# tugitbartlomiej/ViTParticleFilterTracker

Hardware: AMD Instinct MI355X
Metric: frames/sec @ 4096 particles, ViT-B/16 224px; 1/2/4/8 MI355X scaling (higher is better)
Workload: dtype bf16; 1 GPU; 4096 particles, vit_base_patch16_224 bf16, 224x224 frames, full tracking step per frame; particles=4096, particles_per_gpu=4096, arch=vit_base_patch16_224, hip_graph=True, parallelism=particle-shard x1

## Files before the change

### vitparticlefiltertracker_amd/csrc/gemm_bf16.hip

```cpp
#include <algorithm>
#include "gemm_common.h"

using namespace vpf;
using namespace vpf::gemm;

namespace {

constexpr int BK = 64;
constexpr int OPERAND_BYTES = BM * BK * 2;
static_assert(OPERAND_BYTES == TILE_BYTES, "bf16 K-tile geometry");
constexpr int AUX_PARTS = 15;
constexpr int MAX_PARTS = 16;
constexpr int AUX_BYTES = 2048 + AUX_PARTS * 2048;

template <int EPI, bool WIDE = false, bool OUT8 = false, bool PART = false>
__global__ __launch_bounds__(NTHREADS) void k_gemm_bf16(const bf16_t* __restrict__ A, int lda,
                                                        const bf16_t* __restrict__ W,
                                                        const float* __restrict__ bias,
                                                        const bf16_t* residual,
                                                        const float* __restrict__ pos, int g2,
                                                        const float2* __restrict__ stats,
                                                        const float* __restrict__ colsum,
                                                        bf16_t* C, int ldc, int M, int N, int K, int group,
                                                        int stats_parts, float ln_eps, float* stats_out,
                                                        int stats_rows, Out8 o8) {
    constexpr int SMEM = 5 * OPERAND_BYTES;
    static_assert(AUX_BYTES <= OPERAND_BYTES, "aux region must fit the free A slot of the deep ring");
    __shared__ __attribute__((aligned(16))) char smem[SMEM];
    const int tid = threadIdx.x, lane = tid & 63;
    const int wid = __builtin_amdgcn_readfirstlane(tid >> 6);

    int m0, n0;
    tile_of(M, N, group, m0, n0);
    constexpr bool DIRECT = (EPI == VPF_EPI_LN_GELU || EPI == VPF_EPI_BIAS_GELU) && !OUT8 && !PART;

    const int kbase = PART ? (int)blockIdx.y * (K / (int)gridDim.y) : 0;
    const char* Ablk = reinterpret_cast<const char*>(A) + (size_t)m0 * lda * 2 + (size_t)kbase * 2;
    const char* Bblk = reinterpret_cast<const char*>(W) + (size_t)n0 * K * 2 + (size_t)kbase * 2;
    uint32_t offA[4], offB[4];
#pragma unroll
    for (int i = 0; i < 4; ++i) {
        const int g = i * 8 + wid;
        const int row = 8 * g + (lane >> 3);
        const int pch = lane & 7;
        const int lch = pch ^ ((row >> 1) & 7);
        const int ra = min(row, M - 1 - m0);
        const int rb = min(DIRECT ? wperm(row) : row, N - 1 - n0);
        offA[i] = (uint32_t)ra * (uint32_t)(lda * 2) + (uint32_t)(lch * 16);
        offB[i] = (uint32_t)rb * (uint32_t)(K * 2) + (uint32_t)(lch * 16);
    }
    auto stage_a = [&](int kt) {
        char* la = smem + (kt % 3) * OPERAND_BYTES;
        const uint32_t koff = (uint32_t)kt * (BK * 2);
#pragma unroll
        for (int i = 0; i < 4; ++i)
            __builtin_amdgcn_global_load_lds((gptr_t)(Ablk + offA[i] + koff), (lptr_t)(la + (i * 8 + wid) * 1024), 16, 0, 0);
    };
    auto stage_b = [&](int kt) {
        char* lb = smem + (3 + (kt & 1)) * OPERAND_BYTES;
        const uint32_t koff = (uint32_t)kt * (BK * 2);
#pragma unroll
        for (int i = 0; i < 4; ++i)
            __builtin_amdgcn_global_load_lds((gptr_t)(Bblk + offB[i] + koff), (lptr_t)(lb + (i * 8 + wid) * 1024), 16, 0, 0);
    };

    const int wm = wid >> 2, wn = wid & 3;
    f32x4 acc[4][8];
#pragma unroll
    for (int j = 0; j < 4; ++j)
#pragma unroll
        for (int i = 0; i < 8; ++i) acc[j][i] = f32x4{0.f, 0.f, 0.f, 0.f};

    const int fr = lane & 15, fq = lane >> 4;

    constexpr bool LN = (EPI == VPF_EPI_LN || EPI == VPF_EPI_LN_GELU) && !PART;
    const int nk = (PART ? K / (int)gridDim.y : K) / BK;
    char* aux = smem + (nk % 3) * OPERAND_BYTES;
    constexpr bool wide = LN && WIDE;
    char* planes_lds = wide ? smem + ((nk + 1) % 3) * OPERAND_BYTES : aux + 2048;
    auto load_planes = [&](char* dst) {
        const int lane = opaque_lane();
        const float* sd = reinterpret_cast<const float*>(stats);
        const int planes = stats_parts > 0 ? stats_parts : 1;
        if ((M & 1) == 0 && ((uintptr_t)sd & 15) == 0) {
            for (int pc = wid; pc < 2 * planes; pc += 8) {
                const int p = pc >> 1, hf = pc & 1;
                __builtin_amdgcn_global_load_lds(
                    (gptr_t)(sd + (int64_t)p * 2 * M + min(2 * m0 + hf * 256 + lane * 4, 2 * M - 4)),
                    (lptr_t)(dst + p * 2048 + hf * 1024), 16, 0, 0);
            }
        } else {
            for (int p = 0; p < planes; ++p)
                __builtin_amdgcn_global_load_lds(
                    (gptr_t)(sd + (int64_t)p * 2 * M + min(2 * m0 + wid * 64 + lane, 2 * M - 1)),
                    (lptr_t)(dst + p * 2048 + wid * 256), 4, 0, 0);
        }
    };
    auto load_aux = [&]() {
        if constexpr (PART) return;
        const int lane = opaque_lane();
        if (wid == 0)
            __builtin_amdgcn_global_load_lds((gptr_t)(bias + min(n0 + lane * 4, N - 4)), (lptr_t)aux, 16, 0, 0);
        if constexpr (LN) {
            if (wid == 1)
                __builtin_amdgcn_global_load_lds((gptr_t)(colsum + min(n0 + lane * 4, N - 4)), (lptr_t)(aux + 1024), 16,
                                                 0, 0);
            if (!wide) load_planes(aux + 2048);
        }
    };
    stage_a(0);
    stage_b(0);
    if (nk > 1) stage_a(1);
    if (nk == 1) load_aux();
    for (int kt = 0; kt < nk; ++kt) {
        if (kt + 1 < nk) asm volatile("s_waitcnt vmcnt(4)" ::: "memory");
        else asm volatile("s_waitcnt vmcnt(0)" ::: "memory");
        __builtin_amdgcn_s_barrier();
        asm volatile("" ::: "memory");
        if (nk >= 2 && kt == nk - 2) load_aux();
        if (wide && kt == nk - 1) load_planes(planes_lds);
        const char* la = smem + (kt % 3) * OPERAND_BYTES;
        const char* lb = smem + (3 + (kt & 1)) * OPERAND_BYTES;
        bf16x8 a[2][8], b[2][4];
#pragma unroll
        for (int ks = 0; ks < 2; ++ks) {
#pragma unroll
            for (int j = 0; j < 4; ++j) {
                const int row = wn * 64 + j * 16 + fr;
                const int ch = (ks * 4 + fq) ^ ((row >> 1) & 7);
                b[ks][j] = *reinterpret_cast<const bf16x8*>(lb + row * 128 + ch * 16);
            }
#pragma unroll
            for (int i = 0; i < 8; ++i) {
                const int row = wm * 128 + i * 16 + fr;
                const int ch = (ks * 4 + fq) ^ ((row >> 1) & 7);
                a[ks][i] = *reinterpret_cast<const bf16x8*>(la + row * 128 + ch * 16);
            }
        }
        stage_b(min(kt + 1, nk - 1));
        stage_a(min(kt + 2, nk - 1));
#pragma unroll
        for (int ks = 0; ks < 2; ++ks)
#pragma unroll
            for (int j = 0; j < 4; ++j)
#pragma unroll
                for (int i = 0; i < 8; ++i)
                    acc[j][i] = __builtin_amdgcn_mfma_f32_16x16x32_bf16(b[ks][j], a[ks][i], acc[j][i], 0, 0, 0);
        __builtin_amdgcn_sched_group_barrier(0x100, 24, 0);
        __builtin_amdgcn_sched_group_barrier(0x020, 4, 0);
#pragma unroll
        for (int q = 0; q < 4; ++q) {
            __builtin_amdgcn_sched_group_barrier(0x008, 16, 0);
            __builtin_amdgcn_sched_group_barrier(0x020, 1, 0);
        }
    }

    if constexpr (PART) {
        __builtin_amdgcn_s_waitcnt(0x0F70);
        float* P = reinterpret_cast<float*>(C) + (size_t)blockIdx.y * M * N;
#pragma unroll
        for (int i = 0; i < 8; ++i) {
            const int m = m0 + wm * 128 + i * 16 + fr;
#pragma unroll
            for (int j = 0; j < 4; ++j) {
                const int n = n0 + wn * 64 + j * 16 + fq * 4;
                if (m < M && n < N) *reinterpret_cast<f32x4*>(P + (size_t)m * N + n) = acc[j][i];
            }
        }
        return;
    }
    if constexpr (LN) {
        if constexpr (wide) {
            asm volatile("s_waitcnt vmcnt(0)" ::: "memory");
            __builtin_amdgcn_s_barrier();
            asm volatile("" ::: "memory");
        }
        if (stats_parts > 0 && tid < BM) {
            float sm = 0.f, sq = 0.f;
            for (int p = 0; p < stats_parts; ++p) {
                const float2 st = *reinterpret_cast<const float2*>(planes_lds + p * 2048 + tid * 8);
                sm += st.x;
                sq += st.y;
            }
            const float inv_k = 1.0f / (float)K;
            const float mean = sm * inv_k;
            const float var = fmaxf(fmaf(sq, inv_k, -mean * mean), 0.f);
            *reinterpret_cast<float2*>(aux + 2048 + tid * 8) = make_float2(mean, __builtin_amdgcn_rsqf(var + ln_eps));
        }
    }
    __builtin_amdgcn_s_waitcnt(0x0F70);
    uint4 res[16];
    constexpr bool PIPE = EPI != VPF_EPI_PATCH && !OUT8;
    if constexpr (DIRECT) {
        if constexpr (LN) {
            asm volatile("s_waitcnt lgkmcnt(0)" ::: "memory");
            __builtin_amdgcn_s_barrier();
            asm volatile("" ::: "memory");
        }
        store_wave_tile_direct<EPI>(aux, acc, wm, wn, m0, n0, lane, C, ldc, M, N);
        return;
    }
    if constexpr (EPI == VPF_EPI_BIAS_RESIDUAL) load_residual<PIPE>(res, residual, wm, wn, m0, n0, lane, ldc, M, N);
    asm volatile("s_waitcnt lgkmcnt(0)" ::: "memory");
    __builtin_amdgcn_s_barrier();
    asm volatile("" ::: "memory");
    const int region = (wid >> 1) + ((wid >> 1) >= (nk % 3) ? 1 : 0);
    char* img = smem + region * OPERAND_BYTES + (wid & 1) * 16384;
    if constexpr (PIPE) {
        store_wave_tile_pipe<EPI>(img, aux, acc, wm, wn, m0, n0, lane, res, C, ldc, M, N,
                                  EPI == VPF_EPI_BIAS_RESIDUAL ? stats_out : nullptr, stats_rows);
    } else {
        float* prod_stats = (EPI == VPF_EPI_BIAS_RESIDUAL || EPI == VPF_EPI_PATCH) ? stats_out : nullptr;
        store_wave_tile<EPI, OUT8>(img, aux, acc, wm, wn, m0, n0, lane, res, pos, g2, C, ldc, M, N, prod_stats,
                                   stats_rows, o8);
    }
}

template <int EPI, bool OUT8 = false>
__global__ __launch_bounds__(NTHREADS) void k_gemm_pp(const bf16_t* __restrict__ A, int lda,
                                                      const bf16_t* __restrict__ W,
                                                      const float* __restrict__ bias,
                                                      const bf16_t* residual,
                                                      const float* __restrict__ pos, int g2,
                                                      const float2* __restrict__ stats,
                                                      const float* __restrict__ colsum,
                                                      bf16_t* C, int ldc, int M, int N, int K, int group,
                                                      int stats_parts, float ln_eps, float* stats_out,
                                                      int stats_rows, Out8 o8) {
    constexpr int HALF = 16384;
    constexpr int RING = 8 * HALF;
    static_assert(RING + AUX_BYTES <= 160 * 1024, "LDS budget");
    __shared__ __attribute__((aligned(16))) char smem[RING + AUX_BYTES];
    const int tid = threadIdx.x, lane = tid & 63;
    const int wid = __builtin_amdgcn_readfirstlane(tid >> 6);
    const int wm = wid >> 2, wn = wid & 3;

    int m0, n0;
    tile_of(M, N, group, m0, n0);
    constexpr bool DIRECT = (EPI == VPF_EPI_LN_GELU || EPI == VPF_EPI_BIAS_GELU) && !OUT8;

    const char* Ablk = reinterpret_cast<const char*>(A) + (size_t)m0 * lda * 2;
    const char* Bblk = reinterpret_cast<const char*>(W) + (size_t)n0 * K * 2;
    uint32_t off[4][2];
#pragma unroll
    for (int p = 0; p < 2; ++p) {
        const int rho = (wid + 8 * p) * 8 + (lane >> 3);
        const int lch = (lane & 7) ^ ((rho >> 1) & 7);
        const int ra0 = (rho >> 6) * 128 + (rho & 63);
        const int rb0 = (rho >> 5) * 64 + (DIRECT ? wperm(rho & 31) : (rho & 31));
        const int ra[2] = {ra0, ra0 + 64}, rb[2] = {rb0, rb0 + 32};
#pragma unroll
        for (int h = 0; h < 2; ++h) {
            off[h == 0 ? 0 : 3][p] = (uint32_t)min(ra[h], M - 1 - m0) * (uint32_t)(lda * 2) + (uint32_t)(lch * 16);
            off[h == 0 ? 1 : 2][p] = (uint32_t)min(rb[h], N - 1 - n0) * (uint32_t)(K * 2) + (uint32_t)(lch * 16);
        }
    }
    const int nk = K / BK;
    auto stage = [&](int type, int kt) {
        kt = min(kt, nk - 1);
        char* slot = smem + ((kt & 1) * 4 + type) * HALF;
        const char* src = (type == 0 || type == 3) ? Ablk : Bblk;
        const uint32_t koff = (uint32_t)kt * (BK * 2);
#pragma unroll
        for (int p = 0; p < 2; ++p)
            __builtin_amdgcn_global_load_lds((gptr_t)(src + off[type][p] + koff), (lptr_t)(slot + (wid + 8 * p) * 1024),
                                             16, 0, 0);
    };

    constexpr bool LN = (EPI == VPF_EPI_LN || EPI == VPF_EPI_LN_GELU);
    char* aux = smem + RING;
    if (wid == 0)
        __builtin_amdgcn_global_load_lds((gptr_t)(bias + min(n0 + lane * 4, N - 4)), (lptr_t)aux, 16, 0, 0);
    if constexpr (LN) {
        if (wid == 1)
            __builtin_amdgcn_global_load_lds((gptr_t)(colsum + min(n0 + lane * 4, N - 4)), (lptr_t)(aux + 1024), 16, 0, 0);
        const float* sd = reinterpret_cast<const float*>(stats);
        const int planes = stats_parts > 0 ? stats_parts : 1;
        if ((M & 1) == 0 && ((uintptr_t)sd & 15) == 0) {
            for (int pc = wid; pc < 2 * planes; pc += 8) {
                const int p = pc >> 1, hf = pc & 1;
                __builtin_amdgcn_global_load_lds((gptr_t)(sd + (int64_t)p * 2 * M + min(2 * m0 + hf * 256 + lane * 4, 2 * M - 4)),
                                                 (lptr_t)(aux + 2048 + p * 2048 + hf * 1024), 16, 0, 0);
            }
        } else {
            for (int p = 0; p < planes; ++p)
                __builtin_amdgcn_global_load_lds((gptr_t)(sd + (int64_t)p * 2 * M + min(2 * m0 + wid * 64 + lane, 2 * M - 1)),
                                                 (lptr_t)(aux + 2048 + p * 2048 + wid * 256), 4, 0, 0);
        }
    }
    stage(0, 0); stage(1, 0); stage(2, 0); stage(3, 0); stage(0, 1); stage(1, 1);
    asm volatile("s_waitcnt vmcnt(8)" ::: "memory");
    __builtin_amdgcn_s_barrier();
    if (wm == 1) __builtin_amdgcn_s_barrier();
    asm volatile("" ::: "memory");

    f32x4 acc[4][8];
#pragma unroll
    for (int j = 0; j < 4; ++j)
#pragma unroll
        for (int i = 0; i < 8; ++i) acc[j][i] = f32x4{0.f, 0.f, 0.f, 0.f};

    const int fr = lane & 15, fq = lane >> 4;
    const int sw = (fr >> 1) & 7;
    const int abase = (wm * 64 + fr) * 128, bbase = (wn * 32 + fr) * 128;
    auto mfma_quadrant = [&](const i32x4 (&fa)[2][4], const i32x4 (&fb)[2][2], int mh, int nh) {
        asm volatile("s_waitcnt lgkmcnt(0)" ::: "memory");
        __builtin_amdgcn_sched_barrier(0);
#pragma unroll
        for (int ks = 0; ks < 2; ++ks)
#pragma unroll
            for (int j = 0; j < 2; ++j)
#pragma unroll
                for (int i = 0; i < 4; ++i)
                    acc[nh * 2 + j][mh * 4 + i] = __builtin_amdgcn_mfma_f32_16x16x32_bf16(
                        __builtin_bit_cast(bf16x8, fb[ks][j]), __builtin_bit_cast(bf16x8, fa[ks][i]),
                        acc[nh * 2 + j][mh * 4 + i], 0, 0, 0);
        __builtin_amdgcn_sched_barrier(0);
    };
    auto read_a = [&](i32x4 (&fa)[2][4], const char* slot) {
#pragma unroll
        for (int ks = 0; ks < 2; ++ks)
#pragma unroll
            for (int i = 0; i < 4; ++i) fa[ks][i] = lds16(slot + abase + i * 2048 + (((ks * 4 + fq) ^ sw) << 4));
    };
    auto read_b = [&](i32x4 (&fb)[2][2], const char* slot) {
#pragma unroll
        for (int ks = 0; ks < 2; ++ks)
#pragma unroll
            for (int j = 0; j < 2; ++j) fb[ks][j] = lds16(slot + bbase + j * 2048 + (((ks * 4 + fq) ^ sw) << 4));
    };
    auto bar = [&]() {
        __builtin_amdgcn_sched_barrier(0);
        __builtin_amdgcn_s_barrier();
        __builtin_amdgcn_sched_barrier(0);
    };

    for (int kt = 0; kt < nk; ++kt) {
        const char* buf = smem + (kt & 1) * 4 * HALF;
        i32x4 fa0[2][4], fa1[2][4], fb0[2][2], fb1[2][2];
        read_a(fa0, buf);
        read_b(fb0, buf + HALF);
        stage(2, kt + 1);
        asm volatile("s_waitcnt vmcnt(8)" ::: "memory");
        bar();
        mfma_quadrant(fa0, fb0, 0, 0);
        bar();
        read_b(fb1, buf + 2 * HALF);
        stage(3, kt + 1);
        asm volatile("s_waitcnt vmcnt(8)" ::: "memory");
        bar();
        mfma_quadrant(fa0, fb1, 0, 1);
        bar();
        read_a(fa1, buf + 3 * HALF);
        stage(0, kt + 2);
        bar();
        mfma_quadrant(fa1, fb1, 1, 1);
        bar();
        stage(1, kt + 2);
        asm volatile("s_waitcnt vmcnt(8)" ::: "memory");
        bar();
        mfma_quadrant(fa1, fb0, 1, 0);
        bar();
    }
    if (wm == 0) __builtin_amdgcn_s_barrier();
    asm volatile("s_waitcnt vmcnt(0)" ::: "memory");

    if constexpr (LN) {
        if (stats_parts > 0 && tid < BM) {
            float sm = 0.f, sq = 0.f;
            for (int p = 0; p < stats_parts; ++p) {
                const float2 st = *reinterpret_cast<const float2*>(aux + 2048 + p * 2048 + tid * 8);
                sm += st.x;
                sq += st.y;
            }
            const float inv_k = 1.0f / (float)K;
            const float mean = sm * inv_k;
            const float var = fmaxf(fmaf(sq, inv_k, -mean * mean), 0.f);
            *reinterpret_cast<float2*>(aux + 2048 + tid * 8) = make_float2(mean, __builtin_amdgcn_rsqf(var + ln_eps));
        }
    }
    __builtin_amdgcn_s_waitcnt(0x0F70);
    uint4 res[16];
    constexpr bool PIPE = EPI != VPF_EPI_PATCH && !OUT8;
    if constexpr (DIRECT) {
        if constexpr (LN) {
            asm volatile("s_waitcnt lgkmcnt(0)" ::: "memory");
            __builtin_amdgcn_s_barrier();
            asm volatile("" ::: "memory");
        }
        store_wave_tile_direct<EPI>(aux, acc, wm, wn, m0, n0, lane, C, ldc, M, N);
        return;
    }
    if constexpr (EPI == VPF_EPI_BIAS_RESIDUAL) load_residual<PIPE>(res, residual, wm, wn, m0, n0, lane, ldc, M, N);
    asm volatile("s_waitcnt lgkmcnt(0)" ::: "memory");
    __builtin_amdgcn_s_barrier();
    asm volatile("" ::: "memory");
    char* img = smem + wid * 16384;
    if constexpr (PIPE) {
        store_wave_tile_pipe<EPI>(img, aux, acc, wm, wn, m0, n0, lane, res, C, ldc, M, N,
                                  EPI == VPF_EPI_BIAS_RESIDUAL ? stats_out : nullptr, stats_rows);
    } else {
        float* prod_stats = (EPI == VPF_EPI_BIAS_RESIDUAL || EPI == VPF_EPI_PATCH) ? stats_out : nullptr;
        store_wave_tile<EPI, OUT8>(img, aux, acc, wm, wn, m0, n0, lane, res, pos, g2, C, ldc, M, N, prod_stats,
                                   stats_rows, o8);
    }
}

}

#define VPF_IS_LN(E) ((E) == VPF_EPI_LN || (E) == VPF_EPI_LN_GELU)
#define VPF_IS_PROD(E) ((E) == VPF_EPI_BIAS_RESIDUAL || (E) == VPF_EPI_PATCH)
#define VPF_GEMM_ARGS                                                                                        \
    A, (int)lda, W, bias, residual, pos, patch_rows, reinterpret_cast<const float2*>(row_stats), colsum, C,     \
        (int)ldc, m, n, k, group, stats_parts, ln_eps, stats_out, stats_rows, o8
#define VPF_GEMM_LAUNCH(E)                                                                                   \
    do {                                                                                                     \
        if (kern == 5 && !(VPF_IS_LN(E) && stats_parts > AUX_PARTS) && o8.q == nullptr)                      \
            hipLaunchKernelGGL((k_gemm_pp<E, false>), grid, block, 0, s, VPF_GEMM_ARGS);                     \
        else if (kern == 5 && VPF_IS_PROD(E) && o8.q != nullptr)                                             \
            hipLaunchKernelGGL((k_gemm_pp<E, VPF_IS_PROD(E)>), grid, block, 0, s, VPF_GEMM_ARGS);            \
        else if (VPF_IS_LN(E) && stats_parts > AUX_PARTS)                                                    \
            hipLaunchKernelGGL((k_gemm_bf16<E, VPF_IS_LN(E)>), grid, block, 0, s, VPF_GEMM_ARGS);             \
        else if (VPF_IS_PROD(E) && o8.q != nullptr)                                                          \
            hipLaunchKernelGGL((k_gemm_bf16<E, false, VPF_IS_PROD(E)>), grid, block, 0, s, VPF_GEMM_ARGS);    \
        else                                                                                                 \
            hipLaunchKernelGGL((k_gemm_bf16<E>), grid, block, 0, s, VPF_GEMM_ARGS);                           \
    } while (0)

constexpr int kDefaultGroup = 4;
static int g_kernel = 0;
static int g_group = -1;
static int gemm_kernel_for(int epilogue) {
    if (g_kernel) return g_kernel;
    return (epilogue == VPF_EPI_LN || epilogue == VPF_EPI_LN_GELU) ? 5 : 1;
}
static int tile_group_for(int64_t N, int epilogue) {
    if (g_group >= 0) return g_group;
    if (N <= 1024) return 2;
    return epilogue == VPF_EPI_LN_GELU ? 8 : kDefaultGroup;
}
int vpf_gemm_tile_group() { return g_group >= 0 ? g_group : kDefaultGroup; }
int vpf_gemm_tile_group_mx8(int epilogue) {
    if (g_group >= 0) return g_group;
    return epilogue == VPF_EPI_LN ? 8 : kDefaultGroup;
}
VPF_API int vpf_gemm_tune(int kernel, int group) {
    if (kernel != 0 && kernel != 1 && kernel != 5) return VPF_ERR_ARG;
    if (group < -1 || group > 64) return VPF_ERR_ARG;
    g_kernel = kernel;
    g_group = kernel == 0 ? -1 : group;
    return 0;
}

int vpf_check_out8(const uint8_t* C8, int64_t ld8, const uint32_t* Cs, int64_t lds_c, int64_t rows, int64_t N) {
    if (!C8) return Cs ? VPF_ERR_ARG : 0;
    if (!Cs || N % 128 != 0 || ld8 < N || ld8 % 8 != 0 || ((uintptr_t)C8 & 7) || lds_c < rows || lds_c % 64 != 0 ||
        ((uintptr_t)Cs & 3) || ld8 > INT32_MAX || lds_c > INT32_MAX / 4)
        return VPF_ERR_ARG;
    return 0;
}

VPF_API int vpf_gemm_bf16(const uint16_t* A, int64_t lda, const uint16_t* W, const float* bias,
                          const uint16_t* residual, const float* pos, int patch_rows, const float* row_stats,
                          const float* colsum, uint16_t* C, int64_t ldc, int64_t M, int64_t N, int64_t K,
                          int epilogue, int stats_parts, float ln_eps, float* stats_out, uint8_t* C8, int64_t ld8,
                          uint32_t* Cs, int64_t lds_c, void* stream) {
    if (M <= 0 || N <= 0 || K <= 0 || K % BK != 0 || N % 8 != 0 || lda < K || lda % 8 != 0 || ldc < N ||
        ldc % 8 != 0)
        return VPF_ERR_ARG;
    if (M > INT32_MAX / 2 || N > 65536 || K > 65536 || lda > INT32_MAX / 2 || ldc > INT32_MAX / 2) return VPF_ERR_ARG;
    if ((uint64_t)BM * (uint64_t)lda * 2 > UINT32_MAX) return VPF_ERR_ARG;
    if (!A || !W || !bias || !C) return VPF_ERR_ARG;
    if (epilogue == VPF_EPI_BIAS_RESIDUAL && !residual) return VPF_ERR_ARG;
    if (epilogue == VPF_EPI_PATCH && (!pos || patch_rows <= 0 || M % patch_rows != 0)) return VPF_ERR_ARG;
    if ((epilogue == VPF_EPI_LN || epilogue == VPF_EPI_LN_GELU) && (!row_stats || !colsum)) return VPF_ERR_ARG;
    if (((uintptr_t)bias & 15) || ((uintptr_t)colsum & 15) || ((uintptr_t)row_stats & 7)) return VPF_ERR_ARG;
    if (stats_parts < 0 || stats_parts > MAX_PARTS || !(ln_eps >= 0.f))
        return VPF_ERR_ARG;
    if (stats_out && (((uintptr_t)stats_out & 7) || (epilogue != VPF_EPI_BIAS_RESIDUAL && epilogue != VPF_EPI_PATCH)))
        return VPF_ERR_ARG;
    const int64_t srows = epilogue == VPF_EPI_PATCH ? (M / patch_rows) * (patch_rows + 1) : M;
    if (srows > INT32_MAX) return VPF_ERR_ARG;
    const int stats_rows = (int)srows;
    if (C8 && epilogue != VPF_EPI_BIAS_RESIDUAL && epilogue != VPF_EPI_PATCH) return VPF_ERR_ARG;
    if (vpf_check_out8(C8, ld8, Cs, lds_c, srows, N)) return VPF_ERR_ARG;
    const Out8 o8{C8, reinterpret_cast<uint8_t*>(Cs), (int)ld8, (int)lds_c};
    const int64_t tiles = ((M + BM - 1) / BM) * ((N + BN - 1) / BN);
    if (tiles > INT32_MAX) return VPF_ERR_ARG;
    hipStream_t s = (hipStream_t)stream;
    const dim3 grid((unsigned)tiles), block(NTHREADS);
    const int kern = gemm_kernel_for(epilogue);
    const int group = tile_group_for(N, epilogue);
    const int m = (int)M, n = (int)N, k = (int)K;
    switch (epilogue) {
        case VPF_EPI_BIAS: VPF_GEMM_LAUNCH(VPF_EPI_BIAS); break;
        case VPF_EPI_BIAS_GELU: VPF_GEMM_LAUNCH(VPF_EPI_BIAS_GELU); break;
        case VPF_EPI_BIAS_RESIDUAL: VPF_GEMM_LAUNCH(VPF_EPI_BIAS_RESIDUAL); break;
        case VPF_EPI_PATCH: VPF_GEMM_LAUNCH(VPF_EPI_PATCH); break;
        case VPF_EPI_LN: VPF_GEMM_LAUNCH(VPF_EPI_LN); break;
        case VPF_EPI_LN_GELU: VPF_GEMM_LAUNCH(VPF_EPI_LN_GELU); break;
        default: return VPF_ERR_ARG;
    }
    VPF_RETURN_LAUNCH();
}

template <int EPI>
__global__ __launch_bounds__(256) void k_splitk_reduce(const float* __restrict__ P, int S, int M, int N,
                                                       const float* __restrict__ bias,
                                                       const float2* __restrict__ stats,
                                                       const float* __restrict__ colsum, const bf16_t* residual,
                                                       bf16_t* C, int64_t ldc, float* stats_out) {
    constexpr bool LN = (EPI == VPF_EPI_LN || EPI == VPF_EPI_LN_GELU);
    constexpr bool GELU = (EPI == VPF_EPI_BIAS_GELU || EPI == VPF_EPI_LN_GELU);
    const int per_row = N >> 3;
    const int64_t t = (int64_t)blockIdx.x * blockDim.x + threadIdx.x;
    const bool live = t < (int64_t)M * per_row;
    const int m = live ? (int)(t / per_row) : 0;
    const int n = live ? (int)(t - (int64_t)m * per_row) * 8 : 0;
    float v[8];
    if (live) {
        const float* p = P + (size_t)m * N + n;
        const float4 a0 = *reinterpret_cast<const float4*>(p), a1 = *reinterpret_cast<const float4*>(p + 4);
        v[0] = a0.x; v[1] = a0.y; v[2] = a0.z; v[3] = a0.w; v[4] = a1.x; v[5] = a1.y; v[6] = a1.z; v[7] = a1.w;
        for (int s = 1; s < S; ++s) {
            const float* q = p + (size_t)s * M * N;
            const float4 b0 = *reinterpret_cast<const float4*>(q), b1 = *reinterpret_cast<const float4*>(q + 4);
            v[0] += b0.x; v[1] += b0.y; v[2] += b0.z; v[3] += b0.w; v[4] += b1.x; v[5] += b1.y; v[6] += b1.z; v[7] += b1.w;
        }
        float rstd = 1.f, nrm = 0.f;
        if constexpr (LN) {
            const float2 st = stats[m];
            rstd = st.y;
            nrm = -st.y * st.x;
        }
#pragma unroll
        for (int e = 0; e < 8; ++e) {
            float y = LN ? fmaf(rstd, v[e], fmaf(nrm, colsum[n + e], bias[n + e])) : v[e] + bias[n + e];
            if constexpr (GELU) {
                const f32x2 g = gelu_sig2(f32x2{y, y});
                y = g.x;
            }
            v[e] = y;
        }
    }
    uint32_t o[4];
#pragma unroll
    for (int e = 0; e < 4; ++e) o[e] = pack_bf2(v[2 * e], v[2 * e + 1]);
    if constexpr (EPI == VPF_EPI_BIAS_RESIDUAL) {
        if (live) {
            const uint4 rv = *reinterpret_cast<const uint4*>(residual + (size_t)m * ldc + n);
            const uint32_t rr[4] = {rv.x, rv.y, rv.z, rv.w};
#pragma unroll
            for (int e = 0; e < 4; ++e)
                o[e] = pack_bf2(bf2f((bf16_t)(o[e] & 0xffff)) + bf2f((bf16_t)(rr[e] & 0xffff)),
                                bf2f((bf16_t)(o[e] >> 16)) + bf2f((bf16_t)(rr[e] >> 16)));
        }
        if (stats_out != nullptr) {
            float s1 = 0.f, s2 = 0.f;
            if (live) {
#pragma unroll
                for (int e = 0; e < 4; ++e) {
                    const float lo = bf2f((bf16_t)(o[e] & 0xffff)), hi = bf2f((bf16_t)(o[e] >> 16));
                    s1 += lo + hi;
                    s2 = fmaf(lo, lo, s2);
                    s2 = fmaf(hi, hi, s2);
                }
            }
#pragma unroll
            for (int x = 1; x < 8; x <<= 1) {
                s1 += __shfl_xor(s1, x, 64);
                s2 += __shfl_xor(s2, x, 64);
            }
            if (live && (n & 63) == 0)
                *reinterpret_cast<float2*>(stats_out + ((int64_t)(n >> 6) * M + m) * 2) = make_float2(s1, s2);
        }
    }
    if (live) *reinterpret_cast<uint4*>(C + (size_t)m * ldc + n) = make_uint4(o[0], o[1], o[2], o[3]);
}

VPF_API int vpf_gemm_bf16_splitk(const uint16_t* A, int64_t lda, const uint16_t* W, const float* bias,
                                 const uint16_t* residual, const float* row_stats, const float* colsum, uint16_t* C,
                                 int64_t ldc, int64_t M, int64_t N, int64_t K, int epilogue, int splits,
                                 float* stats_out, float* partial_ws, int64_t ws_elems, void* stream) {
    if (M <= 0 || N <= 0 || K <= 0 || splits < 1 || K % ((int64_t)splits * BK) != 0 || N % 8 != 0 || lda < K ||
        lda % 8 != 0 || ldc < N || ldc % 8 != 0)
        return VPF_ERR_ARG;
    if (M > INT32_MAX / 2 || N > 65536 || K > 65536 || lda > INT32_MAX / 2 || ldc > INT32_MAX / 2 || splits > 64)
        return VPF_ERR_ARG;
    if ((uint64_t)BM * (uint64_t)lda * 2 > UINT32_MAX) return VPF_ERR_ARG;
    if (!A || !W || !bias || !C || !partial_ws || ws_elems < (int64_t)splits * M * N) return VPF_ERR_ARG;
    if (((uintptr_t)partial_ws & 15) || ((uintptr_t)C & 15) || ((uintptr_t)A & 15) || ((uintptr_t)W & 15))
        return VPF_ERR_ARG;
    const bool ln = epilogue == VPF_EPI_LN || epilogue == VPF_EPI_LN_GELU;
    if (ln && (!row_stats || !colsum || ((uintptr_t)row_stats & 7))) return VPF_ERR_ARG;
    if (epilogue == VPF_EPI_BIAS_RESIDUAL && (!residual || ((uintptr_t)residual & 15))) return VPF_ERR_ARG;
    if (stats_out && (epilogue != VPF_EPI_BIAS_RESIDUAL || N % 64 != 0 || ((uintptr_t)stats_out & 7)))
        return VPF_ERR_ARG;
    if (epilogue != VPF_EPI_BIAS && epilogue != VPF_EPI_BIAS_GELU && epilogue != VPF_EPI_BIAS_RESIDUAL && !ln)
        return VPF_ERR_ARG;
    const int64_t tiles = ((M + BM - 1) / BM) * ((N + BN - 1) / BN);
    if (tiles > 65535 * 256) return VPF_ERR_ARG;
    hipStream_t s = (hipStream_t)stream;
    const int m = (int)M, n = (int)N, k = (int)K;
    const Out8 o8{nullptr, nullptr, 0, 0};
    hipLaunchKernelGGL((k_gemm_bf16<VPF_EPI_BIAS, false, false, true>),
                       dim3((unsigned)tiles, (unsigned)splits), dim3(NTHREADS), 0, s, reinterpret_cast<const bf16_t*>(A),
                       (int)lda, reinterpret_cast<const bf16_t*>(W), nullptr, nullptr, nullptr, 1, nullptr, nullptr,
                       reinterpret_cast<bf16_t*>(partial_ws), n, m, n, k, vpf_gemm_tile_group(), 0, 0.f, nullptr, m, o8);
    const int e = (int)hipGetLastError();
    if (e) return e;
    const int64_t threads = M * (N / 8);
    const dim3 rg((unsigned)((threads + 255) / 256));
    const float2* st = reinterpret_cast<const float2*>(row_stats);
    const bf16_t* R = reinterpret_cast<const bf16_t*>(residual);
    bf16_t* Cb = reinterpret_cast<bf16_t*>(C);
    switch (epilogue) {
        case VPF_EPI_BIAS:
            hipLaunchKernelGGL(k_splitk_reduce<VPF_EPI_BIAS>, rg, dim3(256), 0, s, partial_ws, splits, m, n, bias, st,
                               colsum, R, Cb, ldc, nullptr);
            break;
        case VPF_EPI_BIAS_GELU:
            hipLaunchKernelGGL(k_splitk_reduce<VPF_EPI_BIAS_GELU>, rg, dim3(256), 0, s, partial_ws, splits, m, n, bias,
                               st, colsum, R, Cb, ldc, nullptr);
            break;
        case VPF_EPI_BIAS_RESIDUAL:
            hipLaunchKernelGGL(k_splitk_reduce<VPF_EPI_BIAS_RESIDUAL>, rg, dim3(256), 0, s, partial_ws, splits, m, n,
                               bias, st, colsum, R, Cb, ldc, stats_out);
            break;
        case VPF_EPI_LN:
            hipLaunchKernelGGL(k_splitk_reduce<VPF_EPI_LN>, rg, dim3(256), 0, s, partial_ws, splits, m, n, bias, st,
                               colsum, R, Cb, ldc, nullptr);
            break;
        default:
            hipLaunchKernelGGL(k_splitk_reduce<VPF_EPI_LN_GELU>, rg, dim3(256), 0, s, partial_ws, splits, m, n, bias,
                               st, colsum, R, Cb, ldc, nullptr);
            break;
    }
    VPF_RETURN_LAUNCH();
}
```

### vitparticlefiltertracker_amd/csrc/gemm_common.h

```cpp
#pragma once
#include "vpf_common.h"
#include "mx8.h"
#include "../../include/vpf.h"

int vpf_gemm_tile_group();
int vpf_gemm_tile_group_mx8(int epilogue);
int vpf_check_out8(const uint8_t* C8, int64_t ld8, const uint32_t* Cs, int64_t lds_c, int64_t rows, int64_t N);

namespace vpf {
namespace gemm {

typedef const __attribute__((address_space(1))) void* gptr_t;
typedef __attribute__((address_space(3))) void* lptr_t;
typedef short bf16x8 __attribute__((ext_vector_type(8)));
typedef int i32x4 __attribute__((ext_vector_type(4)));

__device__ __forceinline__ i32x4 lds16(const char* p) {
    i32x4 v;
    asm volatile("ds_read_b128 %0, %1" : "=v"(v) : "v"((uint32_t)(uintptr_t)(lptr_t)p));
    return v;
}
__device__ __forceinline__ int lds4(const void* p) {
    int v;
    asm volatile("ds_read_b32 %0, %1" : "=v"(v) : "v"((uint32_t)(uintptr_t)(lptr_t)p));
// ... 130 lines not shown
            rsy = f32x2{-st.y * st.x, -st.y * st.x};
        }
#pragma unroll
        for (int j = 0; j < 4; ++j) {
            f32x2 v01, v23;
            const f32x2 a01 = {acc[j][i][0], acc[j][i][1]}, a23 = {acc[j][i][2], acc[j][i][3]};
            const f32x2 b01 = {bv[j].x, bv[j].y}, b23 = {bv[j].z, bv[j].w};
            if constexpr (LN) {
                const f32x2 c01 = {cv[j].x, cv[j].y}, c23 = {cv[j].z, cv[j].w};
                v01 = __builtin_elementwise_fma(rsx, a01, __builtin_elementwise_fma(rsy, c01, b01));
                v23 = __builtin_elementwise_fma(rsx, a23, __builtin_elementwise_fma(rsy, c23, b23));
            } else {
                v01 = a01 + b01;
                v23 = a23 + b23;
            }
            if constexpr (EPI == VPF_EPI_BIAS_GELU || EPI == VPF_EPI_LN_GELU) {
                v01 = gelu_sig2(v01);
                v23 = gelu_sig2(v23);
            }
            const int row = i * 16 + fr;
            const int c8 = (j * 4 + fq) ^ (row & 15);
            *reinterpret_cast<uint2*>(img + row * 128 + c8 * 8) =
                make_uint2(pack_bf2(v01.x, v01.y), pack_bf2(v23.x, v23.y));
        }
        __builtin_amdgcn_wave_barrier();
#pragma unroll
        for (int h = 0; h < 2; ++h) {
            const int row = i * 16 + 2 * (lane >> 3) + h;
            uint4 v = *reinterpret_cast<const uint4*>(img + row * 128 + ((c16 ^ ((row & 15) >> 1)) * 16));
            if (h == 1) { const uint32_t t0 = v.x, t1 = v.y; v.x = v.z; v.y = v.w; v.z = t0; v.w = t1; }
            const int m = m0 + wm * 128 + row;
            const int n = n0 + wn * 64 + c16 * 8;
            const bool ok = m < M && n < N;
            if constexpr (RES) {
                const uint4 rv = res[2 * i + h];
                const uint32_t w[4] = {v.x, v.y, v.z, v.w};
                const uint32_t rr[4] = {rv.x, rv.y, rv.z, rv.w};
                uint32_t o[4];
#pragma unroll
                for (int e = 0; e < 4; ++e)
                    o[e] = pack_bf2(bf2f((bf16_t)(w[e] & 0xffff)) + bf2f((bf16_t)(rr[e] & 0xffff)),
                                    bf2f((bf16_t)(w[e] >> 16)) + bf2f((bf16_t)(rr[e] >> 16)));
                v = make_uint4(o[0], o[1], o[2], o[3]);
                if (stats_out != nullptr) {
                    typedef __bf16 bf16x2_t __attribute__((ext_vector_type(2)));
                    const bf16x2_t one2 = __builtin_bit_cast(bf16x2_t, 0x3F803F80u);
                    float s1 = 0.f, s2 = 0.f;
#pragma unroll
                    for (int e = 0; e < 4; ++e) {
                        const bf16x2_t pr = __builtin_bit_cast(bf16x2_t, o[e]);
                        s1 = __builtin_amdgcn_fdot2_f32_bf16(pr, one2, s1, false);
                        s2 = __builtin_amdgcn_fdot2_f32_bf16(pr, pr, s2, false);
                    }
                    if (!ok) { s1 = 0.f; s2 = 0.f; }
                    *reinterpret_cast<float2*>(img + row * 128 + c16 * 8) = make_float2(s1, s2);
                }
            }
            if (ok) {
                if constexpr (RES) *reinterpret_cast<uint4*>(Cl + (int64_t)(i * 16 + h) * ldc) = v;
                else st16_nt(Cl + (int64_t)(i * 16 + h) * ldc, v);
            }
        }
    }
    if constexpr (RES) {
        const int nb = n0 + wn * 64;
        if (stats_out != nullptr && nb < N) {
            __builtin_amdgcn_wave_barrier();
            float4 t = make_float4(0.f, 0.f, 0.f, 0.f);
#pragma unroll
            for (int q = 0; q < 4; ++q) {
                const float4 u0 = *reinterpret_cast<const float4*>(img + (2 * lane) * 128 + q * 16);
                const float4 u1 = *reinterpret_cast<const float4*>(img + (2 * lane + 1) * 128 + q * 16);
                t.x += u0.x + u0.z; t.y += u0.y + u0.w;
                t.z += u1.x + u1.z; t.w += u1.y + u1.w;
            }
            float* plane = stats_out + (int64_t)(nb >> 6) * stats_rows * 2;
            const int m = m0 + wm * 128 + 2 * lane;
            if (m + 1 < M) *reinterpret_cast<float4*>(plane + (int64_t)m * 2) = t;
            else if (m < M) *reinterpret_cast<float2*>(plane + (int64_t)m * 2) = make_float2(t.x, t.y);
        }
    }
}

__device__ __forceinline__ int wperm(int r) {
    return (r & ~31) | (((r >> 2) & 3) << 3) | (((r >> 4) & 1) << 2) | (r & 3);
}

template <int EPI>
__device__ __forceinline__ void store_wave_tile_direct(const char* aux, const f32x4 (&acc)[4][8], int wm, int wn, int m0,
                                                       int n0, int lane, bf16_t* C, int ldc, int M, int N) {
    static_assert(EPI == VPF_EPI_BIAS_GELU || EPI == VPF_EPI_LN_GELU, "direct stores: the GELU epilogues");
    constexpr bool LN = EPI == VPF_EPI_LN_GELU;
    const int fr = lane & 15, fq = lane >> 4;
    bf16_t* Cl = C + (int64_t)(m0 + wm * 128 + fr) * ldc + (n0 + wn * 64 + fq * 8);
    float4 bv[4], cv[4];
#pragma unroll
    for (int j = 0; j < 4; ++j) {
        const int c = (wn * 64 + (j >> 1) * 32 + fq * 8 + (j & 1) * 4) * 4;
        bv[j] = *reinterpret_cast<const float4*>(aux + c);
        if constexpr (LN) cv[j] = *reinterpret_cast<const float4*>(aux + 1024 + c);
    }
#pragma unroll
    for (int i = 0; i < 8; ++i) {
        f32x2 rsx = {1.f, 1.f}, rsy = {0.f, 0.f};
        if constexpr (LN) {
            const float2 st = *reinterpret_cast<const float2*>(aux + 2048 + (wm * 128 + i * 16 + fr) * 8);
            rsx = f32x2{st.y, st.y};
            rsy = f32x2{-st.y * st.x, -st.y * st.x};
        }
        const int m = m0 + wm * 128 + i * 16 + fr;
#pragma unroll
        for (int h = 0; h < 2; ++h) {
            uint32_t o[4];
#pragma unroll
            for (int k = 0; k < 2; ++k) {
                const int j = 2 * h + k;
                f32x2 v01, v23;
                const f32x2 a01 = {acc[j][i][0], acc[j][i][1]}, a23 = {acc[j][i][2], acc[j][i][3]};
                const f32x2 b01 = {bv[j].x, bv[j].y}, b23 = {bv[j].z, bv[j].w};
                if constexpr (LN) {
                    const f32x2 c01 = {cv[j].x, cv[j].y}, c23 = {cv[j].z, cv[j].w};
                    v01 = __builtin_elementwise_fma(rsx, a01, __builtin_elementwise_fma(rsy, c01, b01));
                    v23 = __builtin_elementwise_fma(rsx, a23, __builtin_elementwise_fma(rsy, c23, b23));
                } else {
                    v01 = a01 + b01;
                    v23 = a23 + b23;
                }
                v01 = gelu_sig2(v01);
                v23 = gelu_sig2(v23);
                o[2 * k] = pack_bf2(v01.x, v01.y);
                o[2 * k + 1] = pack_bf2(v23.x, v23.y);
            }
            const int n = n0 + wn * 64 + h * 32 + fq * 8;
            if (m < M && n < N)
                *reinterpret_cast<uint4*>(Cl + (int64_t)(i * 16) * ldc + h * 32) = make_uint4(o[0], o[1], o[2], o[3]);
        }
    }
}

template <bool PAR = true>
__device__ __forceinline__ void load_residual(uint4 (&res)[16], const bf16_t* residual, int wm, int wn, int m0,
                                              int n0, int lane, int ldc, int M, int N) {
    const int c16 = lane & 7;
    const int n = n0 + wn * 64 + c16 * 8;
    const bf16_t* rl = residual + (int64_t)(m0 + wm * 128 + (PAR ? 2 : 1) * (lane >> 3)) * ldc + n;
#pragma unroll
    for (int it = 0; it < 16; ++it) {
        const int roff = PAR ? (it >> 1) * 16 + (it & 1) : it * 8;
        const int m = m0 + wm * 128 + roff + (PAR ? 2 : 1) * (lane >> 3);
        res[it] = (m < M && n < N) ? *reinterpret_cast<const uint4*>(rl + (int64_t)roff * ldc) : make_uint4(0, 0, 0, 0);
    }
}

template <int EPI, bool OUT8>
__device__ __forceinline__ void store_wave_tile(char* img, const char* aux, const f32x4 (&acc)[4][8], int wm, int wn,
                                                int m0, int n0, int lane, const uint4 (&res)[16],
                                                const float* __restrict__ pos, int g2, bf16_t* C, int ldc, int M,
                                                int N, float* stats_out, int stats_rows, Out8 o8) {
    epi_to_image<EPI>(img, aux, acc, wm, wn, lane);
    const int c16 = lane & 7;
    constexpr bool PROD = (EPI == VPF_EPI_BIAS_RESIDUAL || EPI == VPF_EPI_PATCH);
    constexpr bool GATHER8 = OUT8 && EPI != VPF_EPI_PATCH;
    uint32_t e8s[16];
    __builtin_amdgcn_wave_barrier();
#pragma unroll
    for (int it = 0; it < 16; ++it) {
        const int row = it * 8 + (lane >> 3);
        uint4 v = *reinterpret_cast<const uint4*>(img + row * 128 + ((c16 ^ ((row & 15) >> 1)) * 16));
        if (row & 1) { const uint32_t t0 = v.x, t1 = v.y; v.x = v.z; v.y = v.w; v.z = t0; v.w = t1; }
        const int m = m0 + wm * 128 + row;
        const int n = n0 + wn * 64 + c16 * 8;
        const bool ok = m < M && n < N;
        int64_t orow = m;
        if constexpr (EPI == VPF_EPI_PATCH) {
            const int pi = m % g2;
            orow = (int64_t)(m / g2) * (g2 + 1) + 1 + pi;
            const float* pr = pos + (int64_t)(1 + pi) * N + min(n, N - 8);
            const float4 p0 = *reinterpret_cast<const float4*>(pr);
            const float4 p1 = *reinterpret_cast<const float4*>(pr + 4);
            const uint32_t w[4] = {v.x, v.y, v.z, v.w};
            const float pv[8] = {p0.x, p0.y, p0.z, p0.w, p1.x, p1.y, p1.z, p1.w};
            uint32_t o[4];
#pragma unroll
            for (int e = 0; e < 4; ++e)
                o[e] = pack_bf2(bf2f((bf16_t)(w[e] & 0xffff)) + pv[2 * e], bf2f((bf16_t)(w[e] >> 16)) + pv[2 * e + 1]);
            v = make_uint4(o[0], o[1], o[2], o[3]);
        }
        if constexpr (EPI == VPF_EPI_BIAS_RESIDUAL) {
            const uint4 rv = res[it];
            const uint32_t w[4] = {v.x, v.y, v.z, v.w};
            const uint32_t rr[4] = {rv.x, rv.y, rv.z, rv.w};
            uint32_t o[4];
#pragma unroll
            for (int e = 0; e < 4; ++e)
                o[e] = pack_bf2(bf2f((bf16_t)(w[e] & 0xffff)) + bf2f((bf16_t)(rr[e] & 0xffff)),
                                bf2f((bf16_t)(w[e] >> 16)) + bf2f((bf16_t)(rr[e] >> 16)));
            v = make_uint4(o[0], o[1], o[2], o[3]);
        }
        if constexpr (PROD) {
            if (stats_out != nullptr) {
                typedef __bf16 bf16x2_t __attribute__((ext_vector_type(2)));
                const uint32_t w[4] = {v.x, v.y, v.z, v.w};
                const bf16x2_t one2 = __builtin_bit_cast(bf16x2_t, 0x3F803F80u);
                float s1 = 0.f, s2 = 0.f;
#pragma unroll
                for (int e = 0; e < 4; ++e) {
                    const bf16x2_t pr = __builtin_bit_cast(bf16x2_t, w[e]);
                    s1 = __builtin_amdgcn_fdot2_f32_bf16(pr, one2, s1, false);
                    s2 = __builtin_amdgcn_fdot2_f32_bf16(pr, pr, s2, false);
                }
                if (!ok) { s1 = 0.f; s2 = 0.f; }
                *reinterpret_cast<float2*>(img + row * 128 + c16 * 8) = make_float2(s1, s2);
            }
        }
        if constexpr (OUT8) {
            uint32_t e8;
            const uint2 q = mx8_quant8(v, e8);
            e8s[it] = e8;
            if (ok) {
                *reinterpret_cast<uint2*>(o8.q + orow * o8.ldq + n) = q;
                if (!GATHER8 && (c16 & 3) == 0) o8.s[mx8_scale_byte(orow, n, o8.lds)] = (uint8_t)e8;
            }
        }
        if (ok && C != nullptr) *reinterpret_cast<uint4*>(C + orow * ldc + n) = v;
    }
    if constexpr (GATHER8) {
        __builtin_amdgcn_wave_barrier();
        if ((c16 & 3) == 0) {
#pragma unroll
            for (int it = 0; it < 16; ++it) {
                const int row = it * 8 + (lane >> 3);
                const int w = (row >> 6) * 32 + (c16 >> 2) * 16 + (row & 15);
                img[(w >> 4) * 128 + 64 + (w & 15) * 4 + ((row >> 4) & 3)] = (char)e8s[it];
            }
        }
        __builtin_amdgcn_wave_barrier();
        const uint32_t word = *reinterpret_cast<const uint32_t*>(img + (lane >> 4) * 128 + 64 + (lane & 15) * 4);
        const int nb = n0 + wn * 64;
        const int R = m0 + wm * 128 + (lane >> 5) * 64;
        if (nb < N && R < o8.lds)
            reinterpret_cast<uint32_t*>(o8.s)[(int64_t)(nb >> 7) * o8.lds + R + (((nb >> 5) & 3) + ((lane >> 4) & 1)) * 16 +
                                              (lane & 15)] = word;
    }
    if constexpr (PROD) {
        const int nb = n0 + wn * 64;
        if (stats_out != nullptr && nb < N) {
            __builtin_amdgcn_wave_barrier();
            float4 t = make_float4(0.f, 0.f, 0.f, 0.f);
#pragma unroll
            for (int q = 0; q < 4; ++q) {
                const float4 u0 = *reinterpret_cast<const float4*>(img + (2 * lane) * 128 + q * 16);
                const float4 u1 = *reinterpret_cast<const float4*>(img + (2 * lane + 1) * 128 + q * 16);
                t.x += u0.x + u0.z; t.y += u0.y + u0.w;
                t.z += u1.x + u1.z; t.w += u1.y + u1.w;
            }
            float* plane = stats_out + (int64_t)(nb >> 6) * stats_rows * 2;
            const int m = m0 + wm * 128 + 2 * lane;
            if constexpr (EPI == VPF_EPI_PATCH) {
#pragma unroll
                for (int e = 0; e < 2; ++e) {
                    const int me = m + e;
                    if (me < M) {
                        const int64_t orow = (int64_t)(me / g2) * (g2 + 1) + 1 + me % g2;
                        *reinterpret_cast<float2*>(plane + orow * 2) = e ? make_float2(t.z, t.w) : make_float2(t.x, t.y);
                    }
                }
            } else {
                if (m + 1 < M) *reinterpret_cast<float4*>(plane + (int64_t)m * 2) = t;
                else if (m < M) *reinterpret_cast<float2*>(plane + (int64_t)m * 2) = make_float2(t.x, t.y);
            }
        }
    }
}

__device__ __forceinline__ int wperm16(int r) {
    return (r & ~63) | (((r >> 2) & 3) << 4) | (((r >> 4) & 3) << 2) | (r & 3);
}

template <int EPI>
__device__ __forceinline__ void store_wave_tile_q8_direct(const char* aux, const f32x4 (&acc)[4][8], int wm, int wn,
                                                          int m0, int n0, int lane, int M, int N, Out8 o8) {
    static_assert(EPI == VPF_EPI_LN_GELU, "direct fp8 stores: FC1's epilogue");
    const int fr = lane & 15, fq = lane >> 4;
    float4 bv[4], cv[4];
#pragma unroll
    for (int j = 0; j < 4; ++j) {
        const int c = (wn * 64 + fq * 16 + j * 4) * 4;
        bv[j] = *reinterpret_cast<const float4*>(aux + c);
        cv[j] = *reinterpret_cast<const float4*>(aux + 1024 + c);
    }
    uint32_t word[2] = {0u, 0u};
    const int n = n0 + wn * 64 + fq * 16;
#pragma unroll
    for (int i = 0; i < 8; ++i) {
        const float2 st = *reinterpret_cast<const float2*>(aux + 2048 + (wm * 128 + i * 16 + fr) * 8);
        const f32x2 rsx = {st.y, st.y}, rsy = {-st.y * st.x, -st.y * st.x};
        uint32_t o[8];
#pragma unroll
        for (int j = 0; j < 4; ++j) {
            const f32x2 a01 = {acc[j][i][0], acc[j][i][1]}, a23 = {acc[j][i][2], acc[j][i][3]};
            const f32x2 b01 = {bv[j].x, bv[j].y}, b23 = {bv[j].z, bv[j].w};
            const f32x2 c01 = {cv[j].x, cv[j].y}, c23 = {cv[j].z, cv[j].w};
            f32x2 v01 = __builtin_elementwise_fma(rsx, a01, __builtin_elementwise_fma(rsy, c01, b01));
            f32x2 v23 = __builtin_elementwise_fma(rsx, a23, __builtin_elementwise_fma(rsy, c23, b23));
            v01 = gelu_sig2(v01);
            v23 = gelu_sig2(v23);
// ... 68 lines not shown
```

Before: 7.213 frames/s.

## Prefetch residual tile into LDS via async DMA during final K-steps

```diff
diff --git a/vitparticlefiltertracker_amd/csrc/gemm_bf16.hip b/vitparticlefiltertracker_amd/csrc/gemm_bf16.hip
--- a/vitparticlefiltertracker_amd/csrc/gemm_bf16.hip
+++ b/vitparticlefiltertracker_amd/csrc/gemm_bf16.hip
@@ -1,4 +1,5 @@
 #include <algorithm>
+#include <type_traits>
 #include "gemm_common.h"
 
 using namespace vpf;
@@ -13,7 +14,7 @@
 constexpr int MAX_PARTS = 16;
 constexpr int AUX_BYTES = 2048 + AUX_PARTS * 2048;
 
-template <int EPI, bool WIDE = false, bool OUT8 = false, bool PART = false>
+template <int EPI, bool WIDE = false, bool OUT8 = false, bool PART = false, bool RDMA = false>
 __global__ __launch_bounds__(NTHREADS) void k_gemm_bf16(const bf16_t* __restrict__ A, int lda,
                                                         const bf16_t* __restrict__ W,
                                                         const float* __restrict__ bias,
@@ -26,6 +27,7 @@
                                                         int stats_rows, Out8 o8) {
     constexpr int SMEM = 5 * OPERAND_BYTES;
     static_assert(AUX_BYTES <= OPERAND_BYTES, "aux region must fit the free A slot of the deep ring");
+    static_assert(!RDMA || (EPI == VPF_EPI_BIAS_RESIDUAL && !WIDE && !OUT8 && !PART), "residual DMA: proj / FC2 form");
     __shared__ __attribute__((aligned(16))) char smem[SMEM];
     const int tid = threadIdx.x, lane = tid & 63;
     const int wid = __builtin_amdgcn_readfirstlane(tid >> 6);
@@ -108,12 +110,40 @@
             if (!wide) load_planes(aux + 2048);
         }
     };
+    char* const rd0 = aux + 1024 + wid * 3072;
+    char* const rd1 = smem + ((nk + 1) % 3) * OPERAND_BYTES + wid * 4096;
+    char* const rd2 = smem + (3 + (nk & 1)) * OPERAND_BYTES + wid * 4096;
+    const char* Rblk = reinterpret_cast<const char*>(residual) + (size_t)m0 * ldc * 2;
+    auto stage_res = [&](auto mode_c) {
+        constexpr int MODE = decltype(mode_c)::value;
+        const int lane = opaque_lane();
+        const uint32_t ldc2 = (uint32_t)ldc * 2;
+        const uint32_t rcol = (uint32_t)min(n0 + wn * 64 + (lane & 7) * 8, N - 8) * 2;
+        const uint32_t rv = (uint32_t)(wm * 128 + 2 * (lane >> 3)) * ldc2 + rcol;
+        const uint32_t rlimv = (uint32_t)(M - 1 - m0) * ldc2 + rcol;
+        auto piece = [&](int it, char* dst) {
+            const uint32_t ro = min(rv + (uint32_t)((it >> 1) * 16 + (it & 1)) * ldc2, rlimv);
+            __builtin_amdgcn_global_load_lds((gptr_t)(Rblk + ro), (lptr_t)dst, 16, 0, 0);
+        };
+        if constexpr (MODE == 1) {
+            stage_b(nk - 1);
+#pragma unroll
+            for (int i = 0; i < 3; ++i) piece(i, rd0 + i * 1024);
+        } else {
+#pragma unroll
+            for (int i = 0; i < 4; ++i) piece(3 + i, rd1 + i * 1024);
+#pragma unroll
+            for (int i = 0; i < 4; ++i) piece(7 + i, rd2 + i * 1024);
+        }
+    };
     stage_a(0);
     stage_b(0);
     if (nk > 1) stage_a(1);
     if (nk == 1) load_aux();
-    for (int kt = 0; kt < nk; ++kt) {
-        if (kt + 1 < nk) asm volatile("s_waitcnt vmcnt(4)" ::: "memory");
+    auto kstep = [&](int kt, auto mode_c) {
+        constexpr int MODE = decltype(mode_c)::value;
+        if constexpr (MODE == 2) asm volatile("s_waitcnt vmcnt(3)" ::: "memory");
+        else if (RDMA || kt + 1 < nk) asm volatile("s_waitcnt vmcnt(4)" ::: "memory");
         else asm volatile("s_waitcnt vmcnt(0)" ::: "memory");
         __builtin_amdgcn_s_barrier();
         asm volatile("" ::: "memory");
@@ -122,6 +152,12 @@
         const char* la = smem + (kt % 3) * OPERAND_BYTES;
         const char* lb = smem + (3 + (kt & 1)) * OPERAND_BYTES;
         bf16x8 a[2][8], b[2][4];
+        int fr = lane & 15, fq = lane >> 4;
+        if constexpr (MODE != 0) {
+            const int l = opaque_lane();
+            fr = l & 15;
+            fq = l >> 4;
+        }
 #pragma unroll
         for (int ks = 0; ks < 2; ++ks) {
 #pragma unroll
@@ -137,8 +173,12 @@
                 a[ks][i] = *reinterpret_cast<const bf16x8*>(la + row * 128 + ch * 16);
             }
         }
-        stage_b(min(kt + 1, nk - 1));
-        stage_a(min(kt + 2, nk - 1));
+        if constexpr (MODE == 0) {
+            stage_b(min(kt + 1, nk - 1));
+            stage_a(min(kt + 2, nk - 1));
+        } else {
+            stage_res(mode_c);
+        }
 #pragma unroll
         for (int ks = 0; ks < 2; ++ks)
 #pragma unroll
@@ -149,10 +189,18 @@
         __builtin_amdgcn_sched_group_barrier(0x100, 24, 0);
         __builtin_amdgcn_sched_group_barrier(0x020, 4, 0);
 #pragma unroll
-        for (int q = 0; q < 4; ++q) {
+        for (int q = 0; q < (MODE == 1 ? 3 : 4); ++q) {
             __builtin_amdgcn_sched_group_barrier(0x008, 16, 0);
             __builtin_amdgcn_sched_group_barrier(0x020, 1, 0);
         }
+        if constexpr (MODE != 0) __builtin_amdgcn_sched_barrier(0);
+    };
+    if constexpr (RDMA) {
+        for (int kt = 0; kt < nk - 2; ++kt) kstep(kt, std::integral_constant<int, 0>{});
+        kstep(nk - 2, std::integral_constant<int, 1>{});
+        kstep(nk - 1, std::integral_constant<int, 2>{});
+    } else {
+        for (int kt = 0; kt < nk; ++kt) kstep(kt, std::integral_constant<int, 0>{});
     }
 
     if constexpr (PART) {
@@ -189,6 +237,19 @@
         }
     }
     __builtin_amdgcn_s_waitcnt(0x0F70);
+    (void)stage_res;
+    if constexpr (RDMA) {
+        uint4 rest[16 - RDMA_PIECES];
+        const int lane = opaque_lane();
+        load_residual_rest(rest, residual, wm, wn, m0, n0, lane, ldc, M, N);
+        asm volatile("s_waitcnt lgkmcnt(0)" ::: "memory");
+        __builtin_amdgcn_s_barrier();
+        asm volatile("" ::: "memory");
+        char* img = smem + (wid < 4 ? (nk + 2) % 3 : 3 + ((nk + 1) & 1)) * OPERAND_BYTES + (wid & 3) * 8192;
+        store_wave_tile_pipe_rdma(img, aux, acc, wm, wn, m0, n0, lane, rd0, rd1, rd2, rest, C, ldc, M, N, stats_out,
+                                  stats_rows);
+        return;
+    }
     uint4 res[16];
     constexpr bool PIPE = EPI != VPF_EPI_PATCH && !OUT8;
     if constexpr (DIRECT) {
@@ -495,7 +556,14 @@
     switch (epilogue) {
         case VPF_EPI_BIAS: VPF_GEMM_LAUNCH(VPF_EPI_BIAS); break;
         case VPF_EPI_BIAS_GELU: VPF_GEMM_LAUNCH(VPF_EPI_BIAS_GELU); break;
-        case VPF_EPI_BIAS_RESIDUAL: VPF_GEMM_LAUNCH(VPF_EPI_BIAS_RESIDUAL); break;
+        case VPF_EPI_BIAS_RESIDUAL:
+            if (kern == 1 && o8.q == nullptr && k / BK >= 3 && ((uintptr_t)residual & 15) == 0 &&
+                (uint64_t)BM * (uint64_t)ldc * 2 <= UINT32_MAX)
+                hipLaunchKernelGGL((k_gemm_bf16<VPF_EPI_BIAS_RESIDUAL, false, false, false, true>), grid, block, 0, s,
+                                   VPF_GEMM_ARGS);
+            else
+                VPF_GEMM_LAUNCH(VPF_EPI_BIAS_RESIDUAL);
+            break;
         case VPF_EPI_PATCH: VPF_GEMM_LAUNCH(VPF_EPI_PATCH); break;
         case VPF_EPI_LN: VPF_GEMM_LAUNCH(VPF_EPI_LN); break;
         case VPF_EPI_LN_GELU: VPF_GEMM_LAUNCH(VPF_EPI_LN_GELU); break;
diff --git a/vitparticlefiltertracker_amd/csrc/gemm_common.h b/vitparticlefiltertracker_amd/csrc/gemm_common.h
--- a/vitparticlefiltertracker_amd/csrc/gemm_common.h
+++ b/vitparticlefiltertracker_amd/csrc/gemm_common.h
@@ -306,6 +306,106 @@
     }
 }
 
+constexpr int RDMA_PIECES = 11;
+
+__device__ __forceinline__ void load_residual_rest(uint4 (&rest)[16 - RDMA_PIECES], const bf16_t* residual, int wm,
+                                                   int wn, int m0, int n0, int lane, int ldc, int M, int N) {
+    const int c16 = lane & 7;
+    const int n = n0 + wn * 64 + c16 * 8;
+    const bf16_t* rl = residual + (int64_t)(m0 + wm * 128 + 2 * (lane >> 3)) * ldc + n;
+#pragma unroll
+    for (int it = RDMA_PIECES; it < 16; ++it) {
+        const int roff = (it >> 1) * 16 + (it & 1);
+        const int m = m0 + wm * 128 + roff + 2 * (lane >> 3);
+        rest[it - RDMA_PIECES] =
+            (m < M && n < N) ? *reinterpret_cast<const uint4*>(rl + (int64_t)roff * ldc) : make_uint4(0, 0, 0, 0);
+    }
+}
+
+__device__ __forceinline__ char* rdma_park(char* img, char* rd0, char* rd1, char* rd2, int it) {
+    return it < 3 ? rd0 + it * 1024
+         : it < 7 ? rd1 + (it - 3) * 1024
+         : it < RDMA_PIECES ? rd2 + (it - 7) * 1024
+                            : img + 4096 + (it - RDMA_PIECES) * 512;
+}
+
+__device__ __forceinline__ void store_wave_tile_pipe_rdma(char* img, const char* aux, const f32x4 (&acc)[4][8], int wm,
+                                                          int wn, int m0, int n0, int lane, char* rd0, char* rd1,
+                                                          char* rd2, const uint4 (&rest)[16 - RDMA_PIECES], bf16_t* C,
+                                                          int ldc, int M, int N, float* stats_out, int stats_rows) {
+    const int fr = lane & 15, fq = lane >> 4, c16 = lane & 7, s8 = lane >> 3;
+    bf16_t* Cl = C + (int64_t)(m0 + wm * 128 + 2 * s8) * ldc + (n0 + wn * 64 + c16 * 8);
+    float4 bv[4];
+#pragma unroll
+    for (int j = 0; j < 4; ++j) bv[j] = *reinterpret_cast<const float4*>(aux + (wn * 64 + j * 16 + fq * 4) * 4);
+#pragma unroll
+    for (int i = 0; i < 8; ++i) {
+        char* gi = img + (i & 1) * 2048;
+#pragma unroll
+        for (int j = 0; j < 4; ++j) {
+            const f32x2 a01 = {acc[j][i][0], acc[j][i][1]}, a23 = {acc[j][i][2], acc[j][i][3]};
+            const f32x2 b01 = {bv[j].x, bv[j].y}, b23 = {bv[j].z, bv[j].w};
+            const f32x2 v01 = a01 + b01, v23 = a23 + b23;
+            const int c8 = (j * 4 + fq) ^ fr;
+            *reinterpret_cast<uint2*>(gi + fr * 128 + c8 * 8) = make_uint2(pack_bf2(v01.x, v01.y), pack_bf2(v23.x, v23.y));
+        }
+        __builtin_amdgcn_wave_barrier();
+#pragma unroll
+        for (int h = 0; h < 2; ++h) {
+            const int it = 2 * i + h;
+            const int row = i * 16 + 2 * s8 + h;
+            uint4 v = *reinterpret_cast<const uint4*>(gi + (2 * s8 + h) * 128 + ((c16 ^ s8) * 16));
+            if (h == 1) { const uint32_t t0 = v.x, t1 = v.y; v.x = v.z; v.y = v.w; v.z = t0; v.w = t1; }
+            const int m = m0 + wm * 128 + row;
+            const int n = n0 + wn * 64 + c16 * 8;
+            const bool ok = m < M && n < N;
+            char* park = rdma_park(img, rd0, rd1, rd2, it);
+            const uint4 rv = it < RDMA_PIECES ? *reinterpret_cast<const uint4*>(park + lane * 16)
+                                              : rest[it < RDMA_PIECES ? 0 : it - RDMA_PIECES];
+            const uint32_t w[4] = {v.x, v.y, v.z, v.w};
+            const uint32_t rr[4] = {rv.x, rv.y, rv.z, rv.w};
+            uint32_t o[4];
+#pragma unroll
+            for (int e = 0; e < 4; ++e)
+                o[e] = pack_bf2(bf2f((bf16_t)(w[e] & 0xffff)) + bf2f((bf16_t)(rr[e] & 0xffff)),
+                                bf2f((bf16_t)(w[e] >> 16)) + bf2f((bf16_t)(rr[e] >> 16)));
+            v = make_uint4(o[0], o[1], o[2], o[3]);
+            if (stats_out != nullptr) {
+                typedef __bf16 bf16x2_t __attribute__((ext_vector_type(2)));
+                const bf16x2_t one2 = __builtin_bit_cast(bf16x2_t, 0x3F803F80u);
+                float s1 = 0.f, s2 = 0.f;
+#pragma unroll
+                for (int e = 0; e < 4; ++e) {
+                    const bf16x2_t pr = __builtin_bit_cast(bf16x2_t, o[e]);
+                    s1 = __builtin_amdgcn_fdot2_f32_bf16(pr, one2, s1, false);
+                    s2 = __builtin_amdgcn_fdot2_f32_bf16(pr, pr, s2, false);
+                }
+                if (!ok) { s1 = 0.f; s2 = 0.f; }
+                *reinterpret_cast<float2*>(park + lane * 8) = make_float2(s1, s2);
+            }
+            if (ok) *reinterpret_cast<uint4*>(Cl + (int64_t)(i * 16 + h) * ldc) = v;
+        }
+    }
+    const int nb = n0 + wn * 64;
+    if (stats_out != nullptr && nb < N) {
+        __builtin_amdgcn_wave_barrier();
+        const char* p0 = rdma_park(img, rd0, rd1, rd2, 2 * s8) + c16 * 64;
+        const char* p1 = rdma_park(img, rd0, rd1, rd2, 2 * s8 + 1) + c16 * 64;
+        float4 t = make_float4(0.f, 0.f, 0.f, 0.f);
+#pragma unroll
+        for (int q = 0; q < 4; ++q) {
+            const float4 u0 = *reinterpret_cast<const float4*>(p0 + q * 16);
+            const float4 u1 = *reinterpret_cast<const float4*>(p1 + q * 16);
+            t.x += u0.x + u0.z; t.y += u0.y + u0.w;
+            t.z += u1.x + u1.z; t.w += u1.y + u1.w;
+        }
+        float* plane = stats_out + (int64_t)(nb >> 6) * stats_rows * 2;
+        const int m = m0 + wm * 128 + 2 * lane;
+        if (m + 1 < M) *reinterpret_cast<float4*>(plane + (int64_t)m * 2) = t;
+        else if (m < M) *reinterpret_cast<float2*>(plane + (int64_t)m * 2) = make_float2(t.x, t.y);
+    }
+}
+
 template <int EPI, bool OUT8>
 __device__ __forceinline__ void store_wave_tile(char* img, const char* aux, const f32x4 (&acc)[4][8], int wm, int wn,
                                                 int m0, int n0, int lane, const uint4 (&res)[16],
```

After: 7.269 frames/s, median of 6. About the same (+0.8%).
